# Frank-Wang-oss/GNN_RUL_Benchmarking

Measured on AMD Instinct MI355X. Metric: training samples/sec, C-MAPSS FD004-shaped ST_GCN, higher is better.
Workload: dtype f32 (f16x2-split MFMA operands, fp32 accumulate); 1 GPU; ST_GCN.update (fwd+MSE+bwd+Adam), C-MAPSS FD004-shaped windows [14 sensors x 30], per-GPU batch 65536, dropout 0.2, lr 0.0001, wd 0.0001; per_gpu_batch=65536, global_batch=65536, num_patch=14, patch_size=30, parallelism=dp1, batchnorm=single process, loss_readback=end of run (device-side loss each step)

## Files before the change

gnn_rul_benchmarking_amd/csrc/stgcn_train.hip:

```cpp
#include "stgcn_device.hpp"
#include "stgcn_host.hpp"
#include "stgcn_train_layout.hpp"
#include "stgcn_train_mx.hpp"

namespace rulgnn {


constexpr int TT_STRIDE = 68;
constexpr int TT_ROWS = 30;
constexpr int CONVT_FLOATS = F * 2 * F;
constexpr int BNC = 7;

enum PhaseKind { PH_F = 0, PH_TOP = 1, PH_G = 2 };
constexpr int PHASE_WAVES_F1 = 5, PHASE_WAVES_F2 = 4, PHASE_WAVES_TOP = 3, PHASE_WAVES_G1 = 3, PHASE_WAVES_G0 = 3;

template <int L>
struct SavedSlot {
    static constexpr int X(int l) { return l - 1; }
    static constexpr int H(int l) { return (L - 1) + l; }
    static constexpr int Z1(int l) { return (L - 1) + L + l; }
    static constexpr int O0(int l) { return (L - 1) + 2 * L + l; }
    static constexpr int Z2(int l) { return (L - 1) + 3 * L + l; }
};
static inline int saved_slots(int L) { return 5 * L - 1; }
// ... 1323 lines not shown
    f.gpart = k.gpart; f.cells = k.cells;
    f.grads = a->grads; f.loss = a->loss; f.bn_batch = a->bn_batch;
    f.grid_top = (int)grid;
    for (int i = 0; i < 16; ++i) f.grid_g[i] = (int)grid;
    f.N = k.N; f.L = L; f.K = 1; f.pcount = k.pcount; f.B = s->batch; f.global_batch = a->global_batch;
    f.moment_weight = a->bn_moment_weight;
    f.cell_grad_scale = 1.0f;
    f.guard = 0;
    f.fused_opt = fused_adam ? 1 : 0;
    f.params = fused_adam ? opt->params : nullptr; f.exp_avg = fused_adam ? opt->exp_avg : nullptr;
    f.exp_avg_sq = fused_adam ? opt->exp_avg_sq : nullptr; f.bn_running = fused_adam ? opt->bn_stats : nullptr;
    f.beta1 = fused_adam ? opt->beta1 : 0.f; f.beta2 = fused_adam ? opt->beta2 : 0.f; f.eps = fused_adam ? opt->eps : 0.f;
    f.weight_decay = fused_adam ? opt->weight_decay : 0.f; f.bn_momentum = fused_adam ? opt->bn_momentum : 0.f;
    f.write_grads = 1;
    f.write_loss = (k.has_dpred == 0) && a->loss;
    const float* gy = a->dpred ? a->dpred : a->y;
    if (hipMemsetAsync(c.barrier, 0, sizeof(unsigned), stream) != hipSuccess) return RULGNN_EHIP;
    (void)hipGetLastError();
    hipLaunchKernelGGL(kern, dim3((unsigned)grid), dim3(BLOCK), lds, stream, a->x, a->params, gy, k, c);
    return hipGetLastError() == hipSuccess ? RULGNN_OK : RULGNN_EHIP;
}

template <int RW, int L>
static int run_train_coop(const rulgnn_stgcn_shape* s, const rulgnn_stgcn_train_args* a, hipStream_t stream, const TrainK& k,
                          const WsLayout& w, const TileGeom& g, const rulgnn_adam_args* opt, double bn_count) {
    if constexpr (RW == 16 && L == 2) {
        if (k.N == 14 && k.P == 30) return launch_coop<RW, L, 14, 30>(s, a, stream, k, w, g, opt, bn_count);
        if (k.N == 14 && k.P == 50) return launch_coop<RW, L, 14, 50>(s, a, stream, k, w, g, opt, bn_count);
    }
    return launch_coop<RW, L, 0, 0>(s, a, stream, k, w, g, opt, bn_count);
}

template <int L>
static MxTrainArgs mx_args(const rulgnn_stgcn_shape* s, const rulgnn_stgcn_train_args* a, const TrainK& k, bool wide = false) {
    MxTrainArgs m;
    const size_t tile_floats = wide ? (size_t)F * 64 : (size_t)F * 4 * k.N;
    m.prm = a->params; m.y = a->y; m.pred = a->pred; m.cells = k.cells; m.gpart = k.gpart;
    m.xrec[0] = k.cacheX;
    m.qrec[0] = nullptr;
    for (int l = 0; l < 3; ++l)
        m.mrec[l] = l < L ? reinterpret_cast<uint32_t*>(k.saved + (size_t)SavedSlot<L>::O0(l) * k.ntiles * tile_floats) : nullptr;
    for (int l = 0; l < 3; ++l) m.hrec[l] = l < L ? k.saved + (size_t)SavedSlot<L>::Z1(l) * k.ntiles * tile_floats : nullptr;
    for (int l = 1; l < 3; ++l) {
        m.xrec[l] = l < L ? k.saved + (size_t)SavedSlot<L>::X(l) * k.ntiles * tile_floats : nullptr;
        m.qrec[l] = l < L ? k.saved + (size_t)SavedSlot<L>::Z2(l - 1) * k.ntiles * tile_floats : nullptr;
    }
    m.arec = k.cacheA;
    m.sb = k.sbuf; m.dx = k.rbuf;
    m.dtop = k.saved + (size_t)SavedSlot<L>::H(0) * k.ntiles * tile_floats;
    m.B = s->batch; m.global_batch = a->global_batch; m.sample_offset = a->sample_offset;
    m.N = k.N; m.L = L; m.pcount = k.pcount;
    m.dropout_p = k.dropout_p; m.drop_scale = k.drop_scale; m.drop_thr = k.drop_thr;
    m.do_backward = k.do_backward;
    return m;
}
template <int L>
static int mx_phase(const rulgnn_stgcn_shape* s, const rulgnn_stgcn_train_args* a, const TrainK& k, const MxTrainArgs& m, int ph,
                    hipStream_t stream, int max_grid, int* grid_out, bool wide = false, const HeadScalars* head = nullptr) {
    if (wide) {
        if (ph == 0) return stgcn_train_mxw_f0(m, a->x, s->patch_size, stream, head);
        if (ph < 2 * L) return stgcn_train_mxw_phase(m, PH_F, ph, stream, max_grid, grid_out);
        if (ph == 2 * L) return stgcn_train_mxw_phase(m, PH_TOP, 0, stream, max_grid, grid_out);
        return stgcn_train_mxw_phase(m, PH_G, 4 * L - ph, stream, max_grid, grid_out);
    }
    if (ph == 0)
        return stgcn_train_f0_mx_packed(s, a->x, a->params, m.xrec[0], m.arec, k.cells + cell_fwd(L), cell_stride(L), CELL_REPLICAS, stream, head);
    if (ph < 2 * L) return stgcn_train_mx_phase(m, PH_F, ph, stream, max_grid, grid_out);
    if (ph == 2 * L) return stgcn_train_mx_phase(m, PH_TOP, 0, stream, max_grid, grid_out);
    return stgcn_train_mx_phase(m, PH_G, 4 * L - ph, stream, max_grid, grid_out);
}

template <int RW, int L>
static int run_train_rw(const rulgnn_stgcn_shape* s, const rulgnn_stgcn_train_args* a, int mode, hipStream_t stream,
                        TrainK& k, WsLayout& w, TileGeom& lds, const rulgnn_adam_args* opt, const SyncHook* hook, int path) {
    int rc = RULGNN_OK;
// ... 218 lines not shown
```

gnn_rul_benchmarking_amd/csrc/stgcn_train_mx.hip:

```cpp
#include <algorithm>
#include <cstdlib>
#include <type_traits>

#include "stgcn_host.hpp"
#include "stgcn_mx.hpp"
#include "stgcn_train_layout.hpp"
#include "stgcn_train_mx.hpp"
#include "stgcn_train_mx_ops.hpp"

namespace rulgnn {

#ifdef MXP_TRACE
__device__ unsigned mxp_ts[128];
__device__ int mxp_n;
__device__ unsigned mxp_id[128];
#define MXP_MARKI(ID) do { if (blockIdx.x == 0 && threadIdx.x == 0 && mxp_n < 128) { mxp_id[mxp_n] = ID; mxp_ts[mxp_n++] = (unsigned)wall_clock64(); } } while (0)
#define MXP_MARK() MXP_MARKI(0)
__device__ __forceinline__ void mxp_dump() {
    if (blockIdx.x == 0 && threadIdx.x == 0) {
        for (int i = 0; i < mxp_n; ++i) {
            if (mxp_id[i] >= 100) printf("\nphase %u:", mxp_id[i]);
            else printf(" [%u] +%u", mxp_id[i], mxp_ts[i] - mxp_ts[i - 1]);
        }
        printf("\n");
        mxp_n = 0;
    }
}
#else
#define MXP_MARK() do {} while (0)
#define MXP_MARKI(ID) do {} while (0)
#endif
template <int L, int KIND, int IDX, int NFIX, bool PERSIST>
__device__ __forceinline__ void mxt_phase_body(const MxTrainK& a, float* smem_all, unsigned target) {
    MXP_MARKI(100 + KIND * 10 + IDX);
    const int N = NFIX ? NFIX : a.N;
    const int LS = layer_stride(N);
    const int lane = threadIdx.x & 63, wave = threadIdx.x >> 6;
    const int g = lane >> 4, col = lane & 15;
    constexpr int NBN = 2 * L;
    constexpr int CS = cell_stride(L);
    constexpr int LY = KIND == PH_TOP ? L - 1 : IDX / 2;
    constexpr int BLK = KIND == PH_TOP ? 1 : IDX % 2;
    constexpr bool WITH_PREV = KIND == PH_F && BLK == 0 && LY >= 1;
    constexpr bool BWD_PREV = KIND == PH_G && BLK == 0 && LY >= 1;
    constexpr int LIN = WITH_PREV ? LY - 1 : LY;
    constexpr bool GRAD_IN = KIND == PH_G && (BLK == 1 || LY >= 1);
    constexpr bool GRAD_TOP = GRAD_IN && LY == L - 1;
    constexpr bool NEED_SB = KIND == PH_G && BLK == 0;
    constexpr bool H_OUT = KIND == PH_F && WITH_PREV;
    constexpr bool H_IN = (KIND == PH_F || KIND == PH_G) && BLK == 1 && LY >= 1;
    constexpr bool H_TOP = KIND == PH_TOP && LY >= 1;
    static_assert(!(KIND == PH_F && IDX == 0), "F_0 is stgcn_train_f0_mx_kernel");

    const int XF = 40 * N;
    constexpr int AF = H_IN ? 0 : 220;
    constexpr int SH_BNC = (NBN * MXT_BNC * F + 3) & ~3;
    float* const bnc = smem_all;
    float* const red = smem_all + SH_BNC;
    double* const pairbuf = reinterpret_cast<double*>(red + MXT_RED_FLOATS);
    const int off_zero = 0;
    const int off_scr = off_zero + MXT_ZERO_FLOATS;
    const int off_sh = off_scr + MXT_SCRATCH_FLOATS;
    const int off_wg = off_sh + MXT_SHIFT_FLOATS;
    const int off_X = off_wg + (KIND == PH_G ? MXT_WG_FLOATS : 0);
    const int off_A = off_X + XF;
    const int off_SB = off_A + (H_TOP ? XF : AF);
    const int off_DX = off_SB + (NEED_SB ? XF : 0);
    const int off_XP = off_DX + (GRAD_IN ? XF : 0);
    const int off_HS = off_XP + (BWD_PREV ? XF : 0);
    const int wave_floats = off_HS + (H_OUT ? XF : 0);
    float* const smem = smem_all + SH_BNC + MXT_RED_FLOATS + 2 * MXT_WAVES * (2 * F + 2) + wave * wave_floats;
    u32x2* const sh_tile = reinterpret_cast<u32x2*>(smem + off_sh);
    u32x2* const wg_img = reinterpret_cast<u32x2*>(smem + off_wg);

    int64_t tile = (int64_t)blockIdx.x * MXT_WAVES + wave;
    const int64_t tstride = (int64_t)gridDim.x * MXT_WAVES;

    auto dma = [&](const float* src, int off, int bytes) {
        if constexpr (NFIX != 0) {
            if (bytes == 160 * NFIX) { dma_tile_fixed<160 * NFIX>(src, smem + off, lane); return; }
            if (bytes == 32 * NFIX) { dma_tile_fixed<32 * NFIX>(src, smem + off, lane); return; }
        }
        if constexpr (AF != 0) {
            if (bytes == 4 * AF) { dma_tile_fixed<4 * AF>(src, smem + off, lane); return; }
        }
        dma_tile(src, smem + off, bytes, lane);
    };
    auto req_XA = [&](int64_t t) {
        if constexpr (H_IN) {
            dma(a.hrec[LY] + t * XF, off_X, 4 * XF);
        } else if constexpr (H_TOP) {
            dma(a.xrec[LIN] + t * XF, off_X, 4 * XF);
            dma(a.hrec[LY] + t * XF, off_A, 4 * XF);
        } else {
            dma(a.xrec[LIN] + t * XF, off_X, 4 * XF);
            dma(a.arec + t * AF, off_A, 4 * AF);
        }
    };
    auto req_SB = [&](int64_t t) { if constexpr (NEED_SB) dma(a.sb + t * XF, off_SB, 4 * XF); };
    auto req_DX = [&](int64_t t) {
        if constexpr (GRAD_TOP) dma(a.dtop + t * (8 * N), off_DX, 32 * N);
        else if constexpr (GRAD_IN) dma(a.dx + t * XF, off_DX, 4 * XF);
    };
    auto req_XP = [&](int64_t t) { if constexpr (BWD_PREV) dma(a.qrec[LY] + t * XF, off_XP, 4 * XF); };

    constexpr int FW0 = WITH_PREV ? 2 * LY - 2 : 2 * LY;
    constexpr int NFW = (KIND == PH_F && BLK == 1) || (KIND == PH_G && BLK == 0) ? 1 : 2;
    static_assert(NFW + (KIND == PH_G ? 1 : 0) <= MXT_WAVES, "one reduction pair per wavefront");
    const bool bn_fwd = wave < NFW, bn_mine = bn_fwd || (KIND == PH_G && wave == NFW);
    const int bn_b = bn_fwd ? FW0 + wave : IDX;
    BnPairRaw bnraw;
    if (!PERSIST && bn_mine) bn_pair_load<false>(bnraw, a.cells, a.prm, L, N, bn_fwd, bn_b, lane);
    __builtin_amdgcn_sched_barrier(0);
    for (int i = lane; i < MXT_ZERO_FLOATS; i += 64) smem[off_zero + i] = 0.f;
    if (lane < 2) sh_tile[64 + 65 * lane] = u32x2{0u, 0u};
    if constexpr (KIND == PH_G) {
        if (lane < 2) wg_img[WG_H_HI + WG_ZERO + (WG_H_LO - WG_H_HI) * lane] = u32x2{0u, 0u};
    }
    constexpr int M0_LY = (KIND == PH_F && BLK == 0) ? 1 : 2;
    constexpr int M1_LY = (KIND == PH_F && BLK == 0) ? 0 : ((KIND == PH_F) ? 1 : ((KIND == PH_G && BLK == 0) ? 0 : 2));
    MXP_MARKI(1);
    LayerRaw rc, rp;
    layer_raw(rc, a.prm, LY, N, g, col, M0_LY, M1_LY, !(H_IN || H_TOP));
    if constexpr (WITH_PREV) layer_raw(rp, a.prm, LY - 1, N, g, col, 2, 2);
    ConvOp wT = ConvOp{u32x4{0u, 0u, 0u, 0u}, u32x4{0u, 0u, 0u, 0u}};
    ThetaOp thN = ThetaOp{u32x4{0u, 0u, 0u, 0u}, u32x4{0u, 0u, 0u, 0u}};
    ConvRaw wT_raw = ConvRaw{{0.f, 0.f, 0.f, 0.f}, {0.f, 0.f, 0.f, 0.f}};
    ThetaRaw thN_raw = ThetaRaw{{0.f, 0.f, 0.f, 0.f}};
    if constexpr (KIND == PH_G) {
        wT_raw = conv_bwd_raw(a.prm + LY * LS + off_conv_w(N, BLK), g, col);
        if constexpr (BLK == 0 && LY >= 1) thN_raw = theta_n_raw(a.prm + LY * LS, N, g, col);
    }
    float fc1w[16], fc1wT[16];
    float fc1b = 0.f, fc2w = 0.f, fc2b = 0.f;
    if constexpr (KIND == PH_TOP) {
        const int colc = col < N ? col : 0;
#pragma unroll
        for (int k = 0; k < 16; ++k) {
            const int kc2 = k < N ? k : 0;
            const float v = a.prm[off_fc1_w(N, L) + colc * N + kc2], vt = a.prm[off_fc1_w(N, L) + kc2 * N + colc];
            fc1w[k] = (col < N && k < N) ? v : 0.f;
            fc1wT[k] = (col < N && k < N) ? vt : 0.f;
        }
        const float b1 = a.prm[off_fc1_b(N, L) + colc], w2 = a.prm[off_fc2_w(N, L) + colc];
        fc1b = col < N ? b1 : 0.f;
        fc2w = col < N ? w2 : 0.f;
        fc2b = a.prm[off_fc2_b(N, L)];
    }
    uint32_t dkey[L];
#pragma unroll
    for (int l = 0; l < L; ++l) dkey[l] = step_scratch(a.cells, L)->drop_key[l];
    const bool use_drop = a.dropout_p > 0.f;
    uint32_t mask_next = 0u;
    constexpr bool MASK_IN = KIND == PH_G && BLK == 1;
    if constexpr (MASK_IN) {
        if (use_drop && tile < a.ntiles) mask_next = a.mrec[LY][tile * 64 + lane];
    }
    __builtin_amdgcn_sched_barrier(0);
    if (tile < a.ntiles) { req_XA(tile); req_SB(tile); req_DX(tile); req_XP(tile); }
    {
        MXP_MARKI(2);
        if constexpr (PERSIST) {
            if (threadIdx.x == 0) {
                unsigned* const ctr = step_barrier(a.cells, L);
                unsigned spins = 0;
                while (__hip_atomic_load(ctr, __ATOMIC_RELAXED, __HIP_MEMORY_SCOPE_AGENT) < target) {
                    __builtin_amdgcn_s_sleep(1);
                    if (++spins > (1u << 22)) { atomicOr(&step_scratch(a.cells, L)->pad[0], 4u); break; }
                }
            }
            __syncthreads();
        }
        constexpr bool COH = PERSIST;
        MXP_MARKI(3);
        if (bn_mine) {
            if constexpr (PERSIST) bn_pair_load<COH>(bnraw, a.cells, a.prm, L, N, bn_fwd, bn_b, lane);
            bn_pair_finish(bnraw, bnc, bn_fwd, bn_b, lane);
        }
        if constexpr (KIND == PH_G) {
            wT = conv_bwd_pack(wT_raw);
            if constexpr (BLK == 0 && LY >= 1) thN = theta_pack(thN_raw);
        }
        __syncthreads();
    }
    MXP_MARKI(4);
    LayerK kc;
    layer_constants(kc, rc, bnc, LY, g, col, M0_LY, M1_LY);
    LayerK kp;
    if constexpr (WITH_PREV) layer_constants(kp, rp, bnc, LY - 1, g, col, 2, 2);
    float bA[3] = {0.f, 0.f, 0.f}, bk1[3] = {0.f, 0.f, 0.f}, bk2[3] = {0.f, 0.f, 0.f};
    if constexpr (KIND == PH_G) {
        const float* q = bnc + IDX * MXT_BNC * F;
#pragma unroll
        for (int r = 0; r < 3; ++r) {
            const int c = slot_chan(4 * g + r);
            bA[r] = c >= 0 ? q[4 * F + c] : 0.f;
            bk1[r] = c >= 0 ? q[5 * F + c] * a.gscale : 0.f;
            bk2[r] = c >= 0 ? q[6 * F + c] * a.gscale : 0.f;
        }
    }

    const bool col_ok = col < N;
    const float colm = col_ok ? 1.f : 0.f;
    const int pitch = 4 * N;
    int xoff[3], aoff[3], chan[3];
#pragma unroll
    for (int r = 0; r < 3; ++r) {
        const int c = slot_chan(4 * g + r);
        chan[r] = c;
        xoff[r] = (c >= 0 && col_ok) ? c * pitch + col : -1;
    }
    {
        const int cc = slot_chan(col);
#pragma unroll
        for (int r = 0; r < 3; ++r) {
            const int c = slot_chan(4 * g + r);
            aoff[r] = (c >= 0 && cc >= 0) ? sym(c, cc) : -1;
        }
    }
    auto ld_tile = [&](int base, float (&v)[4][3]) {
#pragma unroll
        for (int s = 0; s < 4; ++s)
// ... 65 lines not shown
        __builtin_amdgcn_sched_barrier(0);
    };
    auto stage_conv = [&](const auto& D, float partner, const ConvOp& w, int rd, int rd_lo, auto& z, auto& keep, auto& keep_sh) {
        constexpr int NS = std::extent_v<std::remove_reference_t<decltype(z)>>;
        u32x4 bh[NS], bl[NS];
#pragma unroll
        for (int s = 0; s < NS; ++s) {
            const Pk p = pack3(D[s][0], D[s][1], D[s][2], partner);
            const Shifted prev = shift_read(sh_tile, rd, rd_lo, lane, p);
            bh[s] = cat(p.hi, prev.hi);
            bl[s] = cat(p.lo, prev.lo);
            keep[s] = p;
            keep_sh[s] = prev;
            __builtin_amdgcn_sched_barrier(0);
        }
        __builtin_amdgcn_sched_barrier(0);
#pragma unroll
        for (int s = 0; s < NS; ++s) {
            z[s] = mfma16z(w.hi, bh[s]);
            z[s] = mfma16(w.hi, bl[s], z[s]);
            z[s] = mfma16(w.lo, bh[s], z[s]);
        }
        __builtin_amdgcn_sched_barrier(0);
    };
    auto leaky_of = [&](const auto& Hp, auto& H) {
        constexpr int NS = std::extent_v<std::remove_reference_t<decltype(H)>>;
#pragma unroll
        for (int s = 0; s < NS; ++s) {
            keep_until_here(Hp[s][3]);
#pragma unroll
            for (int r = 0; r < 3; ++r) H[s][r] = fmaf((1.f - LEAKY) / (1.f + LEAKY), __builtin_fabsf(Hp[s][r]), Hp[s][r]);
        }
    };
    auto layer_full = [&](float (&X)[4][3], const u32x4 (&adjB)[4], const LayerK& k, uint32_t key, const uint32_t (&sbase)[4],
                          float (*xh1_out)[4][3], float (*y2_out)[4][3], float (*q_out)[4][3], uint32_t* mbits_out,
                          const float (*h_in)[4][3] = nullptr) {
        f32x4 z[4];
        float H[4][3], V[4][3];
        Pk pk[4];
        Shifted ps[4];
        if (h_in) {
#pragma unroll
            for (int s = 0; s < 4; ++s)
#pragma unroll
                for (int r = 0; r < 3; ++r) H[s][r] = (*h_in)[s][r];
        } else {
            f32x4 T[4], Hp[4];
            Op2 xo[4];
            stage_T(X, adjB, T, xo);
            stage_Hp(T, k.th, Hp);
            leaky_of(Hp, H);
        }
        stage_conv(H, 1.0f, k.w[0], sh_rd1, sh_rd1_lo, z, pk, ps);
#pragma unroll
        for (int s = 0; s < 4; ++s) {
            keep_until_here(z[s][3]);
#pragma unroll
            for (int r = 0; r < 3; ++r) {
                const float y1 = fmaf(k.gam[0][r], z[s][r], k.bet[0][r]);
                V[s][r] = relu2(fmaf(2.f, H[s][r], relu2(y1)));
            }
        }
        stage_conv(V, 1.0f, k.w[1], sh_rd2, sh_rd2_lo, z, pk, ps);
        uint32_t mbits = 0u;
#pragma unroll
        for (int s = 0; s < 4; ++s) {
            keep_until_here(z[s][3]);
#pragma unroll
            for (int r = 0; r < 3; ++r) {
                const float xh = z[s][r];
                const float y2 = fmaf(k.gam[1][r], xh, k.bet[1][r]);
                if (xh1_out) (*xh1_out)[s][r] = xh;
                if (y2_out) (*y2_out)[s][r] = y2;
                float o1 = fmaf(0.5f, relu2(y2), 0.25f * V[s][r]);
                bool keep = true;
                if (use_drop) {
                    const uint32_t h = lowbias32((sbase[s] + dro[r]) ^ key);
                    keep = h >= a.drop_thr;
                    o1 = keep ? o1 * a.drop_scale : 0.f;
                    mbits |= keep ? 1u << (3 * s + r) : 0u;
                }
                if (q_out) (*q_out)[s][r] = (keep && y2 > 0.f) ? xh : INFINITY;
                X[s][r] = fmaf(colm, o1, X[s][r]);
            }
        }
        *mbits_out = mbits;
    };

    bool pend = false;
    int64_t pend_tile = 0;
    int pend_ns = 0;
    float pend_v[4][3], pend_q[4][3], pend_h[4][3];
    float pend_top0 = 0.f, pend_top1 = 0.f, pend_pred = 0.f;
    uint32_t pend_m = 0u;
#pragma unroll
    for (int s = 0; s < 4; ++s)
#pragma unroll
        for (int r = 0; r < 3; ++r) pend_v[s][r] = pend_q[s][r] = pend_h[s][r] = 0.f;

    MXP_MARKI(5);
    for (; tile < a.ntiles; tile += tstride) {
        const int64_t s0 = tile * 4;
        const int ns_tile = (int)((a.B - s0) < 4 ? (a.B - s0) : 4);
        auto tile_body = [&](auto FULL_) {
        constexpr bool FULL = decltype(FULL_)::value;
        const int ns = FULL ? 4 : ns_tile;
        const int64_t nt = tile + tstride;
        asm volatile("s_waitcnt vmcnt(0) lgkmcnt(0)" ::: "memory");
        __builtin_amdgcn_wave_barrier();
        if (!pend) MXP_MARKI(13);
        if (pend) {
            if constexpr (WITH_PREV) {
                st_tile(a.xrec[LY] + pend_tile * XF, pend_v, pend_ns);
                st_tile(a.qrec[LY] + pend_tile * XF, pend_q, pend_ns);
                if (use_drop) a.mrec[LY - 1][pend_tile * 64 + lane] = pend_m;
            }
            if constexpr (H_OUT) st_tile_staged(a.hrec[LY] + pend_tile * XF, pend_h);
            if constexpr (KIND == PH_G && BLK == 1) st_tile(a.sb + pend_tile * XF, pend_v, pend_ns);
            if constexpr (BWD_PREV) st_tile(a.dx + pend_tile * XF, pend_v, pend_ns);
            if constexpr (KIND == PH_TOP) {
                if (g < pend_ns && col_ok && a.do_backward) {
                    float* p = a.dtop + pend_tile * (8 * N) + g * N + col;
                    p[0] = pend_top0;
                    p[pitch] = pend_top1;
                }
                if (g < pend_ns && col == 0) a.pred[pend_tile * 4 + g] = pend_pred;
                if (use_drop && a.do_backward) a.mrec[LY][pend_tile * 64 + lane] = pend_m;
            }
        }
        float X[4][3];
        float HT[4][3];
        u32x4 adjB[4];
        ld_tile(off_X, X);
        if constexpr (H_TOP) ld_tile(off_A, HT);
        if constexpr (H_IN || H_TOP) {
            if (ns < 4) {
#pragma unroll
                for (int s = 0; s < 4; ++s)
                    if (s >= ns) {
                        X[s][0] = X[s][1] = X[s][2] = 0.f;
                        if constexpr (H_TOP) HT[s][0] = HT[s][1] = HT[s][2] = 0.f;
                    }
            }
        } else {
#pragma unroll
            for (int s = 0; s < 4; ++s) {
                unsigned q[3];
#pragma unroll
                for (int r = 0; r < 3; ++r) q[r] = __builtin_bit_cast(unsigned, smem[(aoff[r] >= 0 ? off_A + aoff[r] : off_zero) + s * 55]);
                adjB[s] = u32x4{__builtin_amdgcn_perm(q[1], q[0], 0x05040100u), q[2] & 0xFFFFu, __builtin_amdgcn_perm(q[1], q[0], 0x07060302u), q[2] >> 16};
            }
            if (ns < 4) {
#pragma unroll
                for (int s = 0; s < 4; ++s)
                    if (s >= ns) { adjB[s] = u32x4{0u, 0u, 0u, 0u}; X[s][0] = X[s][1] = X[s][2] = 0.f; }
            }
        }
        asm volatile("s_waitcnt lgkmcnt(0)" ::: "memory");
        __builtin_amdgcn_wave_barrier();
        if (nt < a.ntiles) req_XA(nt);
        uint32_t sbase[4];
#pragma unroll
        for (int s = 0; s < 4; ++s) sbase[s] = (uint32_t)((a.sample_offset + s0 + s) * F) * (uint32_t)N;
        const bool any_row = true;
        (void)any_row;

        if constexpr (KIND == PH_F) {
            if constexpr (WITH_PREV) {
                layer_full(X, adjB, kp, dkey[LY - 1], sbase, nullptr, nullptr, &pend_q, &pend_m);
#pragma unroll
                for (int s = 0; s < 4; ++s)
#pragma unroll
                    for (int r = 0; r < 3; ++r) pend_v[s][r] = X[s][r];
            }
            f32x4 z[4];
            float H[4][3];
            Pk pk[4];
            Shifted ps[4];
            if constexpr (H_IN) {
#pragma unroll
                for (int s = 0; s < 4; ++s)
#pragma unroll
                    for (int r = 0; r < 3; ++r) H[s][r] = X[s][r];
            } else {
                f32x4 T[4], Hp[4];
                Op2 xo[4];
                stage_T(X, adjB, T, xo);
                stage_Hp(T, kc.th, Hp);
                leaky_of(Hp, H);
            }
            if constexpr (H_OUT) {
#pragma unroll
                for (int s = 0; s < 4; ++s)
#pragma unroll
                    for (int r = 0; r < 3; ++r) pend_h[s][r] = H[s][r];
            }
            if constexpr (BLK == 0) {
                stage_conv(H, 0.f, kc.w[0], sh_rd1, sh_rd1_lo, z, pk, ps);
            } else {
                stage_conv(H, 1.0f, kc.w[0], sh_rd1, sh_rd1_lo, z, pk, ps);
                float V[4][3];
#pragma unroll
                for (int s = 0; s < 4; ++s) {
                    keep_until_here(z[s][3]);
#pragma unroll
                    for (int r = 0; r < 3; ++r) V[s][r] = relu2(fmaf(2.f, H[s][r], relu2(fmaf(kc.gam[0][r], z[s][r], kc.bet[0][r]))));
                }
                stage_conv(V, 0.f, kc.w[1], sh_rd2, sh_rd2_lo, z, pk, ps);
            }
#pragma unroll
            for (int s = 0; s < 4; ++s) {
                keep_until_here(z[s][3]);
                if (s < ns) {
#pragma unroll
                    for (int r = 0; r < 3; ++r) {
                        const float zv = z[s][r] * colm;
                        s_a[r] += zv;
                        s_b[r] = fmaf(zv, zv, s_b[r]);
                    }
                }
            }
            if constexpr (H_OUT) { pend = true; pend_tile = tile; pend_ns = ns; }
            return;
        }

        if constexpr (KIND == PH_TOP) {
            float xh1[4][3], y2[4][3];
            const float ylab = a.y[s0 + (g < ns ? g : ns - 1)];
            if constexpr (H_TOP) layer_full(X, adjB, kc, dkey[LY], sbase, &xh1, &y2, nullptr, &pend_m, &HT);
            else layer_full(X, adjB, kc, dkey[LY], sbase, &xh1, &y2, nullptr, &pend_m);
            float pm[4], pa[4];
#pragma unroll
            for (int s = 0; s < 4; ++s) {
                const float v0 = X[s][0], v1 = g == 3 ? X[s][0] : X[s][1], v2 = g == 3 ? X[s][0] : X[s][2];
                float m = v0;
                int ar = 0;
                if (v1 > m) { m = v1; ar = 1; }
                if (v2 > m) { m = v2; ar = 2; }
                pm[s] = fmaf(v0 + v1 + v2, 0.f, m);
                pa[s] = __builtin_bit_cast(float, 3 * g + ar);
            }
            transpose_rows4(pm[0], pm[1], pm[2], pm[3]);
            transpose_rows4(pa[0], pa[1], pa[2], pa[3]);
            float pooled = pm[0];
            int arg = __builtin_bit_cast(int, pa[0]);
#pragma unroll
            for (int q = 1; q < 4; ++q) {
                const bool take = pm[q] > pooled;
                pooled = take ? pm[q] : pooled;
                arg = take ? __builtin_bit_cast(int, pa[q]) : arg;
            }
            pooled = fmaf((pm[0] + pm[1]) + (pm[2] + pm[3]), 0.f, pooled);
            const bool rowok = g < ns, valid = rowok && col_ok;
            pooled = valid ? pooled : 0.f;
            float y1 = fc1b;
            fmac1_rowbcast<0>(y1, pooled, fc1w[0]);   fmac1_rowbcast<1>(y1, pooled, fc1w[1]);   fmac1_rowbcast<2>(y1, pooled, fc1w[2]);
            fmac1_rowbcast<3>(y1, pooled, fc1w[3]);   fmac1_rowbcast<4>(y1, pooled, fc1w[4]);   fmac1_rowbcast<5>(y1, pooled, fc1w[5]);
            fmac1_rowbcast<6>(y1, pooled, fc1w[6]);   fmac1_rowbcast<7>(y1, pooled, fc1w[7]);   fmac1_rowbcast<8>(y1, pooled, fc1w[8]);
            fmac1_rowbcast<9>(y1, pooled, fc1w[9]);   fmac1_rowbcast<10>(y1, pooled, fc1w[10]); fmac1_rowbcast<11>(y1, pooled, fc1w[11]);
            fmac1_rowbcast<12>(y1, pooled, fc1w[12]); fmac1_rowbcast<13>(y1, pooled, fc1w[13]); fmac1_rowbcast<14>(y1, pooled, fc1w[14]);
            fmac1_rowbcast<15>(y1, pooled, fc1w[15]);
            y1 = relu(y1);
            const float pred = Row<16>::allsum(y1 * fc2w) + fc2b;
// ... 255 lines not shown
                        for (int e = 0; e < NS; ++e) {
                            keep_until_here(dXl[e][3]);
#pragma unroll
                            for (int r = 0; r < 3; ++r) {
                                const float dX = (HS + e < ns) ? (dXl[e][r] + gin[HS + e][r]) * colm : 0.f;
                                pend_v[HS + e][r] = dX;
                                const bool open = Q[HS + e][r] < INFINITY;
                                const float dy = open ? dX * a.drop_scale : 0.f;
                                s_a[r] += dy;
                                s_b[r] = fmaf(dy, open ? Q[HS + e][r] : 0.f, s_b[r]);
                            }
                        }
                    }
                }
            };
            g_half(std::integral_constant<int, 0>{});
            __builtin_amdgcn_sched_barrier(0);
            g_half(std::integral_constant<int, 2>{});
            if constexpr (BLK == 1 || LY >= 1) { pend = true; pend_tile = tile; pend_ns = ns; }
        }
        };
        if (ns_tile == 4) tile_body(std::true_type{});
        else tile_body(std::false_type{});
    }

    MXP_MARKI(6);
    if (pend) {
        if constexpr (WITH_PREV) {
            st_tile(a.xrec[LY] + pend_tile * XF, pend_v, pend_ns);
            st_tile(a.qrec[LY] + pend_tile * XF, pend_q, pend_ns);
            if (use_drop) a.mrec[LY - 1][pend_tile * 64 + lane] = pend_m;
        }
        if constexpr (H_OUT) st_tile_staged(a.hrec[LY] + pend_tile * XF, pend_h);
        if constexpr (KIND == PH_G && BLK == 1) st_tile(a.sb + pend_tile * XF, pend_v, pend_ns);
        if constexpr (BWD_PREV) st_tile(a.dx + pend_tile * XF, pend_v, pend_ns);
        if constexpr (KIND == PH_TOP) {
            if (g < pend_ns && col_ok && a.do_backward) {
                float* p = a.dtop + pend_tile * (8 * N) + g * N + col;
                p[0] = pend_top0;
                p[pitch] = pend_top1;
            }
            if (g < pend_ns && col == 0) a.pred[pend_tile * 4 + g] = pend_pred;
            if (use_drop && a.do_backward) a.mrec[LY][pend_tile * 64 + lane] = pend_m;
        }
    }

    MXP_MARKI(7);
    StepScratch* const sc = step_scratch(a.cells, L);
    bool bad = false;
    const bool has_pair = (KIND == PH_F) || (KIND == PH_TOP && a.do_backward) || (KIND == PH_G && IDX > 0);
    constexpr int PBW = 2 * F + 2;
    if (has_pair) {
#pragma unroll
        for (int r = 0; r < 3; ++r) {
            double da = (double)s_a[r], db = (double)s_b[r];
#pragma unroll
            for (int off = 8; off >= 1; off >>= 1) {
                da += __shfl_xor(da, off, 16);
                db += __shfl_xor(db, off, 16);
            }
            if (col == 0 && chan[r] >= 0) {
                pairbuf[wave * PBW + chan[r]] = da;
                pairbuf[wave * PBW + F + chan[r]] = db;
            }
        }
    }
// ... 104 lines not shown
    asm volatile("s_waitcnt vmcnt(0) lgkmcnt(0)" ::: "memory");
    MXP_MARKI(12);
    __syncthreads();
    if (threadIdx.x == 0) __hip_atomic_fetch_add(step_barrier(a.cells, L), 1u, __ATOMIC_RELAXED, __HIP_MEMORY_SCOPE_AGENT);
    ++arrived_phases;
}
template <int L, int NFIX, int I>
struct MxtPersistChain {
    static __device__ __forceinline__ void forward(const MxTrainK& a, float* smem_all, unsigned& n) {
        if constexpr (I > 1) MxtPersistChain<L, NFIX, I - 1>::forward(a, smem_all, n);
        mxt_persist_phase<L, PH_F, I, NFIX>(a, smem_all, n);
    }
    static __device__ __forceinline__ void backward(const MxTrainK& a, float* smem_all, unsigned& n) {
        mxt_persist_phase<L, PH_G, I, NFIX>(a, smem_all, n);
        if constexpr (I > 0) MxtPersistChain<L, NFIX, I - 1>::backward(a, smem_all, n);
    }
};
template <int L, int NFIX>
__global__ __launch_bounds__(64 * MXT_WAVES, MX_WAVES_PER_SIMD) void stgcn_train_mx_persist_kernel(MxTrainK a) {
    extern __shared__ __attribute__((aligned(16))) float smem_all[];
    unsigned n = 0;
    MxtPersistChain<L, NFIX, 2 * L - 1>::forward(a, smem_all, n);
    mxt_persist_phase<L, PH_TOP, 0, NFIX>(a, smem_all, n);
    MxtPersistChain<L, NFIX, 2 * L - 1>::backward(a, smem_all, n);
#ifdef MXP_TRACE
    mxp_dump();
#endif
}

static constexpr size_t mxt_lds_bytes(int L, int kind, int idx, int N) {
    const int blk = kind == PH_TOP ? 1 : idx % 2, ly = kind == PH_TOP ? L - 1 : idx / 2;
    const bool need_sb = kind == PH_G && blk == 0, grad_in = kind == PH_G && (blk == 1 || ly >= 1), bwd_prev = kind == PH_G && blk == 0 && ly >= 1;
    const bool h_in = (kind == PH_F || kind == PH_G) && blk == 1 && ly >= 1;
    const bool h_top = kind == PH_TOP && ly >= 1;
    const bool h_out = kind == PH_F && blk == 0 && ly >= 1;
    const int XF = 40 * N;
    const size_t wave = (size_t)MXT_ZERO_FLOATS + MXT_SCRATCH_FLOATS + MXT_SHIFT_FLOATS + (kind == PH_G ? MXT_WG_FLOATS : 0) + XF + (h_in ? 0 : h_top ? XF : 220) + (need_sb ? XF : 0) + (grad_in ? XF : 0) +
                        (bwd_prev ? XF : 0) + (h_out ? XF : 0);
    const size_t shared = (size_t)((2 * L * MXT_BNC * F + 3) & ~3) + MXT_RED_FLOATS + 2 * MXT_WAVES * (2 * F + 2);
    return (shared + MXT_WAVES * wave) * sizeof(float);
}
constexpr size_t MXT_MAX_LDS_BYTES = 80 * 1024;
static_assert(mxt_lds_bytes(MX_MAX_LAYERS, PH_G, 2, 15) <= MXT_MAX_LDS_BYTES && mxt_lds_bytes(MX_MAX_LAYERS, PH_G, 3, 15) <= MXT_MAX_LDS_BYTES,
              "the largest matrix-core phase must fit its LDS limit");

template <int L, int KIND, int IDX, int NFIX>
static int mxt_launch(const MxTrainK& k, hipStream_t stream, int max_grid, int* grid_out) {
    auto kern = &stgcn_train_mx_kernel<L, KIND, IDX, NFIX>;
    const size_t lds = mxt_lds_bytes(L, KIND, IDX, k.N);
    if (lds > MXT_MAX_LDS_BYTES) return RULGNN_EUNSUPPORTED;
    if (lds > 48 * 1024 &&
        hipFuncSetAttribute(reinterpret_cast<const void*>(kern), hipFuncAttributeMaxDynamicSharedMemorySize, (int)lds) != hipSuccess)
        return RULGNN_EHIP;
    int dev = 0, cus = 256, per_cu = 0;
    if (hipGetDevice(&dev) == hipSuccess) {
        int v = 0;
        if (hipDeviceGetAttribute(&v, hipDeviceAttributeMultiprocessorCount, dev) == hipSuccess && v > 0) cus = v;
    }
    if (hipOccupancyMaxActiveBlocksPerMultiprocessor(&per_cu, kern, 64 * MXT_WAVES, lds) != hipSuccess || per_cu < 1) per_cu = 1;
    if (per_cu > MX_WAVES_PER_SIMD) per_cu = MX_WAVES_PER_SIMD;
    if (const char* e = getenv("RULGNN_MXT_BLOCKS_PER_CU")) { const int v = atoi(e); if (v > 0) per_cu = v; }
    int64_t grid = (int64_t)cus * per_cu;
    const int64_t want = (k.ntiles + MXT_WAVES - 1) / MXT_WAVES;
    if (grid > want) grid = want;
    if (grid > max_grid) grid = max_grid;
    if (grid_out) *grid_out = (int)grid;
    (void)hipGetLastError();
    hipLaunchKernelGGL(kern, dim3((unsigned)grid), dim3(64 * MXT_WAVES), lds, stream, k);
    return hipGetLastError() == hipSuccess ? RULGNN_OK : RULGNN_EHIP;
}

// ... 4 lines not shown
}

template <int L, int I>
struct MxtPhase {
    static int run(int kind, int idx, const MxTrainK& k, hipStream_t st, int mg, int* go) {
        if (idx == I) {
            if (kind == PH_F) {
                if constexpr (I >= 1) return mxt_launch_n<L, PH_F, I>(k, st, mg, go);
                else return RULGNN_EINVAL;
            }
            if (kind == PH_G) return mxt_launch_n<L, PH_G, I>(k, st, mg, go);
        }
        if constexpr (I > 0) return MxtPhase<L, I - 1>::run(kind, idx, k, st, mg, go);
        return RULGNN_EINVAL;
    }
};

bool stgcn_train_mx_shape_ok(const rulgnn_stgcn_shape* s, const float* x) {
    const int N = s->num_patch, P = s->patch_size, L = s->num_layers;
    if (N < 2 || N > 15 || L < 1 || L > MX_MAX_LAYERS || s->mpnn_k != 1) return false;
    if (((int64_t)N * P) % 4 != 0 || (reinterpret_cast<uintptr_t>(x) & 15) != 0) return false;
    return true;
}

float stgcn_train_mx_grad_scale(int64_t global_batch) {
    int e = 0;
    while (((int64_t)1 << e) < global_batch && e < 40) ++e;
    return ldexpf(1.0f, e + 3);
}

static MxTrainK mxt_kernel_args(const MxTrainArgs& m) {
    MxTrainK k;
    k.prm = m.prm; k.y = m.y; k.pred = m.pred; k.cells = m.cells; k.gpart = m.gpart;
    for (int l = 0; l < MX_MAX_LAYERS; ++l) { k.xrec[l] = m.xrec[l]; k.qrec[l] = m.qrec[l]; k.hrec[l] = m.hrec[l]; k.mrec[l] = m.mrec[l]; }
    k.arec = m.arec; k.sb = m.sb; k.dx = m.dx; k.dtop = m.dtop;
    k.B = m.B; k.ntiles = (m.B + 3) / 4; k.global_batch = m.global_batch; k.sample_offset = m.sample_offset;
    k.N = m.N; k.pcount = m.pcount;
    k.dropout_p = m.dropout_p; k.drop_scale = m.drop_scale; k.drop_thr = m.drop_thr;
    k.gscale = stgcn_train_mx_grad_scale(m.global_batch);
    k.inv_gscale = 1.0f / k.gscale;
    k.do_backward = m.do_backward;
    return k;
}

template <int NFIX>
static int mxt_persist_launch(const MxTrainK& k, hipStream_t stream, int64_t grid) {
    constexpr int L = 2;
    auto kern = &stgcn_train_mx_persist_kernel<L, NFIX>;
    size_t lds = 0;
    for (int i = 1; i < 2 * L; ++i) lds = std::max(lds, mxt_lds_bytes(L, PH_F, i, k.N));
    lds = std::max(lds, mxt_lds_bytes(L, PH_TOP, 0, k.N));
    for (int i = 0; i < 2 * L; ++i) lds = std::max(lds, mxt_lds_bytes(L, PH_G, i, k.N));
    if (lds > MXT_MAX_LDS_BYTES) return RULGNN_EUNSUPPORTED;
    if (lds > 48 * 1024 &&
        hipFuncSetAttribute(reinterpret_cast<const void*>(kern), hipFuncAttributeMaxDynamicSharedMemorySize, (int)lds) != hipSuccess)
        return RULGNN_EHIP;
    (void)hipGetLastError();
    hipLaunchKernelGGL(kern, dim3((unsigned)grid), dim3(64 * MXT_WAVES), lds, stream, k);
    return hipGetLastError() == hipSuccess ? RULGNN_OK : RULGNN_EHIP;
}
int stgcn_train_mx_persistent_grid(int64_t batch, int num_layers, int max_grid) {
    if (num_layers != 2 || batch <= 0) return 0;
    int dev = 0, cus = 256;
    if (hipGetDevice(&dev) == hipSuccess) {
        int v = 0;
        if (hipDeviceGetAttribute(&v, hipDeviceAttributeMultiprocessorCount, dev) == hipSuccess && v > 0) cus = v;
    }
// ... 33 lines not shown
```

gnn_rul_benchmarking_amd/csrc/stgcn_train_mx.hpp:

```cpp
#pragma once
#include <hip/hip_runtime.h>
#include <stdint.h>

#include "../../include/rulgnn.h"

namespace rulgnn {

struct MxTrainArgs {
    const float* prm;
    const float* y;
    float* pred;
    double* cells;
    float* gpart;
    float* xrec[3];
    float* qrec[3];
    float* hrec[3];
    uint32_t* mrec[3];
    float* arec;
    float* sb;
    float* dx;
    float* dtop;
    int64_t B, global_batch, sample_offset;
    int N, L, pcount;
    float dropout_p, drop_scale;
    uint32_t drop_thr;
    int do_backward;
};

bool stgcn_train_mx_shape_ok(const rulgnn_stgcn_shape* s, const float* x);
float stgcn_train_mx_grad_scale(int64_t global_batch);
int stgcn_train_mx_phase(const MxTrainArgs& m, int kind, int idx, hipStream_t stream, int max_grid, int* grid_out);
int stgcn_train_mx_persistent_grid(int64_t batch, int num_layers, int max_grid);
int stgcn_train_mx_persistent(const MxTrainArgs& m, hipStream_t stream, int max_grid, int* grid_out);
struct HeadScalars;
int stgcn_train_f0_mx_packed(const rulgnn_stgcn_shape* s, const float* x, const float* prm, float* xrec0, float* arec, double* cells_bn0,
                             int cell_stride_doubles, int replicas, hipStream_t stream, const HeadScalars* head = nullptr);


bool stgcn_train_mxw_shape_ok(const rulgnn_stgcn_shape* s, const float* x);
int stgcn_train_mxw_f0(const MxTrainArgs& m, const float* x, int patch_size, hipStream_t stream, const HeadScalars* head = nullptr);
int stgcn_train_mxw_phase(const MxTrainArgs& m, int kind, int idx, hipStream_t stream, int max_grid, int* grid_out);

}
```

gnn_rul_benchmarking_amd/csrc/stgcn_train_mx_ops.hpp:

```cpp
#pragma once
#include <type_traits>

#include "stgcn_mx.hpp"
#include "stgcn_train_layout.hpp"

namespace rulgnn {
namespace {

constexpr int MXT_ZERO_FLOATS = 192;
constexpr int MXT_SCRATCH_FLOATS = 128;
constexpr int MXT_SHIFT_FLOATS = 264;
constexpr int WG_ZERO = 64;
constexpr int WG_DZ_HI = 0, WG_DZ_LO = 64, WG_H_HI = 128, WG_H_LO = WG_H_HI + 65;
constexpr int MXT_WG_FLOATS = (2 * (WG_H_LO + 65) + 3) & ~3;
constexpr int MXT_WAVES = 4;
constexpr int MXT_RED_FLOATS = 448;
constexpr int MXT_BNC = BN_TABLE_ROWS;

enum { PH_F = 0, PH_TOP = 1, PH_G = 2 };

struct Op2 { u32x4 h, l; };
struct Pk { u32x2 hi, lo; };

__device__ __forceinline__ Pk pack3(float a, float b, float c, float d) {
// ... 117 lines not shown
    }
}
__device__ __forceinline__ void layer_constants(LayerK& k, const LayerRaw& raw, const float* bnc, int l, int g, int col, int mode0, int mode1) {
    k.th = theta_pack(raw.th);
    const int co = slot_chan(col), coc = co >= 0 ? co : 0;
#pragma unroll
    for (int blk = 0; blk < 2; ++blk) {
        const int mode = blk == 0 ? mode0 : mode1;
        const float* q = bnc + (2 * l + blk) * MXT_BNC * F;
        const float istd = mode == 2 ? q[1 * F + coc] : 1.f;
        const float shift = mode == 2 ? -q[0 * F + coc] * istd : 0.f;
        if (mode != 0) k.w[blk] = conv_fwd_operand(raw.w[blk], istd, shift, blk == 0 ? 1.f : 0.25f, g, col);
        else k.w[blk] = ConvOp{u32x4{0u, 0u, 0u, 0u}, u32x4{0u, 0u, 0u, 0u}};
#pragma unroll
        for (int r = 0; r < 3; ++r) {
            const int c = slot_chan(4 * g + r);
            k.gam[blk][r] = (mode == 2 && c >= 0) ? q[2 * F + c] : 0.f;
            k.bet[blk][r] = (mode == 2 && c >= 0) ? q[3 * F + c] : 0.f;
        }
    }
}

}

struct MxTrainK {
    const float* prm;
    const float* y;
    float* pred;
    double* cells;
    float* gpart;
    float* xrec[MX_MAX_LAYERS];
    float* qrec[MX_MAX_LAYERS];
    float* hrec[MX_MAX_LAYERS];
    uint32_t* mrec[MX_MAX_LAYERS];
    float* arec;
    float* sb;
    float* dx;
    float* dtop;
    int64_t B, ntiles, global_batch, sample_offset;
    int N, pcount;
    float dropout_p, drop_scale;
    uint32_t drop_thr;
    float gscale, inv_gscale;
    int do_backward;
};

}
```

Measured before the change: 207.5 million samples/s.

## Store block-1 conv input per layer and reload it instead of recomputing

```diff
diff --git a/gnn_rul_benchmarking_amd/csrc/stgcn_train.hip b/gnn_rul_benchmarking_amd/csrc/stgcn_train.hip
--- a/gnn_rul_benchmarking_amd/csrc/stgcn_train.hip
+++ b/gnn_rul_benchmarking_amd/csrc/stgcn_train.hip
@@ -1379,6 +1379,21 @@
 }
 
 template <int L>
+constexpr int mx_orec_slot(int l) { return l < L - 1 ? SavedSlot<L>::H(l + 1) : SavedSlot<L>::Z2(L - 1); }
+template <int L>
+constexpr bool mx_orec_slots_free() {
+    for (int l = 0; l < L; ++l) {
+        const int v = mx_orec_slot<L>(l);
+        if (v < 0 || v >= 5 * L - 1 || v == SavedSlot<L>::H(0)) return false;
+        for (int j = 0; j < L; ++j) {
+            if (v == SavedSlot<L>::Z1(j) || v == SavedSlot<L>::O0(j) || (j != l && v == mx_orec_slot<L>(j))) return false;
+            if (j >= 1 && (v == SavedSlot<L>::X(j) || v == SavedSlot<L>::Z2(j - 1))) return false;
+        }
+    }
+    return true;
+}
+static_assert(mx_orec_slots_free<1>() && mx_orec_slots_free<2>() && mx_orec_slots_free<3>(), "the o0 record must not share a slot");
+template <int L>
 static MxTrainArgs mx_args(const rulgnn_stgcn_shape* s, const rulgnn_stgcn_train_args* a, const TrainK& k, bool wide = false) {
     MxTrainArgs m;
     const size_t tile_floats = wide ? (size_t)F * 64 : (size_t)F * 4 * k.N;
@@ -1388,6 +1403,7 @@
     for (int l = 0; l < 3; ++l)
         m.mrec[l] = l < L ? reinterpret_cast<uint32_t*>(k.saved + (size_t)SavedSlot<L>::O0(l) * k.ntiles * tile_floats) : nullptr;
     for (int l = 0; l < 3; ++l) m.hrec[l] = l < L ? k.saved + (size_t)SavedSlot<L>::Z1(l) * k.ntiles * tile_floats : nullptr;
+    for (int l = 0; l < 3; ++l) m.orec[l] = (l < L && !wide) ? k.saved + (size_t)mx_orec_slot<L>(l) * k.ntiles * tile_floats : nullptr;
     for (int l = 1; l < 3; ++l) {
         m.xrec[l] = l < L ? k.saved + (size_t)SavedSlot<L>::X(l) * k.ntiles * tile_floats : nullptr;
         m.qrec[l] = l < L ? k.saved + (size_t)SavedSlot<L>::Z2(l - 1) * k.ntiles * tile_floats : nullptr;
diff --git a/gnn_rul_benchmarking_amd/csrc/stgcn_train_mx.hip b/gnn_rul_benchmarking_amd/csrc/stgcn_train_mx.hip
--- a/gnn_rul_benchmarking_amd/csrc/stgcn_train_mx.hip
+++ b/gnn_rul_benchmarking_amd/csrc/stgcn_train_mx.hip
@@ -49,7 +49,8 @@
     constexpr bool NEED_SB = KIND == PH_G && BLK == 0;
     constexpr bool H_OUT = KIND == PH_F && WITH_PREV;
     constexpr bool H_IN = (KIND == PH_F || KIND == PH_G) && BLK == 1 && LY >= 1;
-    constexpr bool H_TOP = KIND == PH_TOP && LY >= 1;
+    constexpr bool V_OUT = KIND == PH_F && BLK == 1;
+    constexpr bool V_TOP = KIND == PH_TOP;
     static_assert(!(KIND == PH_F && IDX == 0), "F_0 is stgcn_train_f0_mx_kernel");
 
     const int XF = 40 * N;
@@ -64,11 +65,12 @@
     const int off_wg = off_sh + MXT_SHIFT_FLOATS;
     const int off_X = off_wg + (KIND == PH_G ? MXT_WG_FLOATS : 0);
     const int off_A = off_X + XF;
-    const int off_SB = off_A + (H_TOP ? XF : AF);
+    const int off_SB = off_A + (V_TOP ? XF : AF);
     const int off_DX = off_SB + (NEED_SB ? XF : 0);
     const int off_XP = off_DX + (GRAD_IN ? XF : 0);
-    const int off_HS = off_XP + (BWD_PREV ? XF : 0);
-    const int wave_floats = off_HS + (H_OUT ? XF : 0);
+    const int off_V = off_XP + (BWD_PREV ? XF : 0);
+    const int off_HS = off_V + (WITH_PREV ? XF : 0);
+    const int wave_floats = off_HS + ((H_OUT || V_OUT) ? XF : 0);
     float* const smem = smem_all + SH_BNC + MXT_RED_FLOATS + 2 * MXT_WAVES * (2 * F + 2) + wave * wave_floats;
     u32x2* const sh_tile = reinterpret_cast<u32x2*>(smem + off_sh);
     u32x2* const wg_img = reinterpret_cast<u32x2*>(smem + off_wg);
@@ -89,12 +91,13 @@
     auto req_XA = [&](int64_t t) {
         if constexpr (H_IN) {
             dma(a.hrec[LY] + t * XF, off_X, 4 * XF);
-        } else if constexpr (H_TOP) {
+        } else if constexpr (V_TOP) {
             dma(a.xrec[LIN] + t * XF, off_X, 4 * XF);
-            dma(a.hrec[LY] + t * XF, off_A, 4 * XF);
+            dma(a.orec[LY] + t * XF, off_A, 4 * XF);
         } else {
             dma(a.xrec[LIN] + t * XF, off_X, 4 * XF);
             dma(a.arec + t * AF, off_A, 4 * AF);
+            if constexpr (WITH_PREV) dma(a.orec[LIN] + t * XF, off_V, 4 * XF);
         }
     };
     auto req_SB = [&](int64_t t) { if constexpr (NEED_SB) dma(a.sb + t * XF, off_SB, 4 * XF); };
@@ -104,8 +107,8 @@
     };
     auto req_XP = [&](int64_t t) { if constexpr (BWD_PREV) dma(a.qrec[LY] + t * XF, off_XP, 4 * XF); };
 
-    constexpr int FW0 = WITH_PREV ? 2 * LY - 2 : 2 * LY;
-    constexpr int NFW = (KIND == PH_F && BLK == 1) || (KIND == PH_G && BLK == 0) ? 1 : 2;
+    constexpr int FW0 = WITH_PREV ? 2 * LY - 1 : (V_TOP ? 2 * LY + 1 : 2 * LY);
+    constexpr int NFW = KIND == PH_G && BLK == 1 ? 2 : 1;
     static_assert(NFW + (KIND == PH_G ? 1 : 0) <= MXT_WAVES, "one reduction pair per wavefront");
     const bool bn_fwd = wave < NFW, bn_mine = bn_fwd || (KIND == PH_G && wave == NFW);
     const int bn_b = bn_fwd ? FW0 + wave : IDX;
@@ -117,12 +120,12 @@
     if constexpr (KIND == PH_G) {
         if (lane < 2) wg_img[WG_H_HI + WG_ZERO + (WG_H_LO - WG_H_HI) * lane] = u32x2{0u, 0u};
     }
-    constexpr int M0_LY = (KIND == PH_F && BLK == 0) ? 1 : 2;
+    constexpr int M0_LY = (KIND == PH_F && BLK == 0) ? 1 : (V_TOP ? 0 : 2);
     constexpr int M1_LY = (KIND == PH_F && BLK == 0) ? 0 : ((KIND == PH_F) ? 1 : ((KIND == PH_G && BLK == 0) ? 0 : 2));
     MXP_MARKI(1);
     LayerRaw rc, rp;
-    layer_raw(rc, a.prm, LY, N, g, col, M0_LY, M1_LY, !(H_IN || H_TOP));
-    if constexpr (WITH_PREV) layer_raw(rp, a.prm, LY - 1, N, g, col, 2, 2);
+    layer_raw(rc, a.prm, LY, N, g, col, M0_LY, M1_LY, !(H_IN || V_TOP));
+    if constexpr (WITH_PREV) layer_raw(rp, a.prm, LY - 1, N, g, col, 0, 2, false);
     ConvOp wT = ConvOp{u32x4{0u, 0u, 0u, 0u}, u32x4{0u, 0u, 0u, 0u}};
     ThetaOp thN = ThetaOp{u32x4{0u, 0u, 0u, 0u}, u32x4{0u, 0u, 0u, 0u}};
     ConvRaw wT_raw = ConvRaw{{0.f, 0.f, 0.f, 0.f}, {0.f, 0.f, 0.f, 0.f}};
@@ -187,7 +190,7 @@
     LayerK kc;
     layer_constants(kc, rc, bnc, LY, g, col, M0_LY, M1_LY);
     LayerK kp;
-    if constexpr (WITH_PREV) layer_constants(kp, rp, bnc, LY - 1, g, col, 2, 2);
+    if constexpr (WITH_PREV) layer_constants(kp, rp, bnc, LY - 1, g, col, 0, 2);
     float bA[3] = {0.f, 0.f, 0.f}, bk1[3] = {0.f, 0.f, 0.f}, bk2[3] = {0.f, 0.f, 0.f};
     if constexpr (KIND == PH_G) {
         const float* q = bnc + IDX * MXT_BNC * F;
@@ -319,35 +322,11 @@
             for (int r = 0; r < 3; ++r) H[s][r] = fmaf((1.f - LEAKY) / (1.f + LEAKY), __builtin_fabsf(Hp[s][r]), Hp[s][r]);
         }
     };
-    auto layer_full = [&](float (&X)[4][3], const u32x4 (&adjB)[4], const LayerK& k, uint32_t key, const uint32_t (&sbase)[4],
-                          float (*xh1_out)[4][3], float (*y2_out)[4][3], float (*q_out)[4][3], uint32_t* mbits_out,
-                          const float (*h_in)[4][3] = nullptr) {
+    auto layer_tail = [&](float (&X)[4][3], const float (&V)[4][3], const LayerK& k, uint32_t key, const uint32_t (&sbase)[4],
+                          float (*xh1_out)[4][3], float (*y2_out)[4][3], float (*q_out)[4][3], uint32_t* mbits_out) {
         f32x4 z[4];
-        float H[4][3], V[4][3];
         Pk pk[4];
         Shifted ps[4];
-        if (h_in) {
-#pragma unroll
-            for (int s = 0; s < 4; ++s)
-#pragma unroll
-                for (int r = 0; r < 3; ++r) H[s][r] = (*h_in)[s][r];
-        } else {
-            f32x4 T[4], Hp[4];
-            Op2 xo[4];
-            stage_T(X, adjB, T, xo);
-            stage_Hp(T, k.th, Hp);
-            leaky_of(Hp, H);
-        }
-        stage_conv(H, 1.0f, k.w[0], sh_rd1, sh_rd1_lo, z, pk, ps);
-#pragma unroll
-        for (int s = 0; s < 4; ++s) {
-            keep_until_here(z[s][3]);
-#pragma unroll
-            for (int r = 0; r < 3; ++r) {
-                const float y1 = fmaf(k.gam[0][r], z[s][r], k.bet[0][r]);
-                V[s][r] = relu2(fmaf(2.f, H[s][r], relu2(y1)));
-            }
-        }
         stage_conv(V, 1.0f, k.w[1], sh_rd2, sh_rd2_lo, z, pk, ps);
         uint32_t mbits = 0u;
 #pragma unroll
@@ -403,6 +382,7 @@
                 if (use_drop) a.mrec[LY - 1][pend_tile * 64 + lane] = pend_m;
             }
             if constexpr (H_OUT) st_tile_staged(a.hrec[LY] + pend_tile * XF, pend_h);
+            if constexpr (V_OUT) st_tile_staged(a.orec[LY] + pend_tile * XF, pend_h);
             if constexpr (KIND == PH_G && BLK == 1) st_tile(a.sb + pend_tile * XF, pend_v, pend_ns);
             if constexpr (BWD_PREV) st_tile(a.dx + pend_tile * XF, pend_v, pend_ns);
             if constexpr (KIND == PH_TOP) {
@@ -416,18 +396,23 @@
             }
         }
         float X[4][3];
-        float HT[4][3];
+        float VR[4][3];
         u32x4 adjB[4];
         ld_tile(off_X, X);
-        if constexpr (H_TOP) ld_tile(off_A, HT);
-        if constexpr (H_IN || H_TOP) {
+        if constexpr (V_TOP) ld_tile(off_A, VR);
+        if constexpr (WITH_PREV) ld_tile(off_V, VR);
+        if constexpr (V_TOP || WITH_PREV) {
             if (ns < 4) {
 #pragma unroll
                 for (int s = 0; s < 4; ++s)
-                    if (s >= ns) {
-                        X[s][0] = X[s][1] = X[s][2] = 0.f;
-                        if constexpr (H_TOP) HT[s][0] = HT[s][1] = HT[s][2] = 0.f;
-                    }
+                    if (s >= ns) VR[s][0] = VR[s][1] = VR[s][2] = 0.f;
+            }
+        }
+        if constexpr (H_IN || V_TOP) {
+            if (ns < 4) {
+#pragma unroll
+                for (int s = 0; s < 4; ++s)
+                    if (s >= ns) X[s][0] = X[s][1] = X[s][2] = 0.f;
             }
         } else {
 #pragma unroll
@@ -454,7 +439,7 @@
 
         if constexpr (KIND == PH_F) {
             if constexpr (WITH_PREV) {
-                layer_full(X, adjB, kp, dkey[LY - 1], sbase, nullptr, nullptr, &pend_q, &pend_m);
+                layer_tail(X, VR, kp, dkey[LY - 1], sbase, nullptr, nullptr, &pend_q, &pend_m);
 #pragma unroll
                 for (int s = 0; s < 4; ++s)
 #pragma unroll
@@ -491,7 +476,7 @@
                 for (int s = 0; s < 4; ++s) {
                     keep_until_here(z[s][3]);
 #pragma unroll
-                    for (int r = 0; r < 3; ++r) V[s][r] = relu2(fmaf(2.f, H[s][r], relu2(fmaf(kc.gam[0][r], z[s][r], kc.bet[0][r]))));
+                    for (int r = 0; r < 3; ++r) pend_h[s][r] = V[s][r] = relu2(fmaf(2.f, H[s][r], relu2(fmaf(kc.gam[0][r], z[s][r], kc.bet[0][r]))));
                 }
                 stage_conv(V, 0.f, kc.w[1], sh_rd2, sh_rd2_lo, z, pk, ps);
             }
@@ -507,15 +492,14 @@
                     }
                 }
             }
-            if constexpr (H_OUT) { pend = true; pend_tile = tile; pend_ns = ns; }
+            if constexpr (H_OUT || V_OUT) { pend = true; pend_tile = tile; pend_ns = ns; }
             return;
         }
 
         if constexpr (KIND == PH_TOP) {
             float xh1[4][3], y2[4][3];
             const float ylab = a.y[s0 + (g < ns ? g : ns - 1)];
-            if constexpr (H_TOP) layer_full(X, adjB, kc, dkey[LY], sbase, &xh1, &y2, nullptr, &pend_m, &HT);
-            else layer_full(X, adjB, kc, dkey[LY], sbase, &xh1, &y2, nullptr, &pend_m);
+            layer_tail(X, VR, kc, dkey[LY], sbase, &xh1, &y2, nullptr, &pend_m);
             float pm[4], pa[4];
 #pragma unroll
             for (int s = 0; s < 4; ++s) {
@@ -837,6 +821,7 @@
             if (use_drop) a.mrec[LY - 1][pend_tile * 64 + lane] = pend_m;
         }
         if constexpr (H_OUT) st_tile_staged(a.hrec[LY] + pend_tile * XF, pend_h);
+        if constexpr (V_OUT) st_tile_staged(a.orec[LY] + pend_tile * XF, pend_h);
         if constexpr (KIND == PH_G && BLK == 1) st_tile(a.sb + pend_tile * XF, pend_v, pend_ns);
         if constexpr (BWD_PREV) st_tile(a.dx + pend_tile * XF, pend_v, pend_ns);
         if constexpr (KIND == PH_TOP) {
@@ -1007,11 +992,12 @@
     const int blk = kind == PH_TOP ? 1 : idx % 2, ly = kind == PH_TOP ? L - 1 : idx / 2;
     const bool need_sb = kind == PH_G && blk == 0, grad_in = kind == PH_G && (blk == 1 || ly >= 1), bwd_prev = kind == PH_G && blk == 0 && ly >= 1;
     const bool h_in = (kind == PH_F || kind == PH_G) && blk == 1 && ly >= 1;
-    const bool h_top = kind == PH_TOP && ly >= 1;
-    const bool h_out = kind == PH_F && blk == 0 && ly >= 1;
+    const bool v_top = kind == PH_TOP;
+    const bool with_prev = kind == PH_F && blk == 0 && ly >= 1;
+    const bool v_out = kind == PH_F && blk == 1;
     const int XF = 40 * N;
-    const size_t wave = (size_t)MXT_ZERO_FLOATS + MXT_SCRATCH_FLOATS + MXT_SHIFT_FLOATS + (kind == PH_G ? MXT_WG_FLOATS : 0) + XF + (h_in ? 0 : h_top ? XF : 220) + (need_sb ? XF : 0) + (grad_in ? XF : 0) +
-                        (bwd_prev ? XF : 0) + (h_out ? XF : 0);
+    const size_t wave = (size_t)MXT_ZERO_FLOATS + MXT_SCRATCH_FLOATS + MXT_SHIFT_FLOATS + (kind == PH_G ? MXT_WG_FLOATS : 0) + XF + (h_in ? 0 : v_top ? XF : 220) + (need_sb ? XF : 0) + (grad_in ? XF : 0) +
+                        (bwd_prev ? XF : 0) + (with_prev ? 2 * XF : 0) + (v_out ? XF : 0);
     const size_t shared = (size_t)((2 * L * MXT_BNC * F + 3) & ~3) + MXT_RED_FLOATS + 2 * MXT_WAVES * (2 * F + 2);
     return (shared + MXT_WAVES * wave) * sizeof(float);
 }
@@ -1082,7 +1068,7 @@
 static MxTrainK mxt_kernel_args(const MxTrainArgs& m) {
     MxTrainK k;
     k.prm = m.prm; k.y = m.y; k.pred = m.pred; k.cells = m.cells; k.gpart = m.gpart;
-    for (int l = 0; l < MX_MAX_LAYERS; ++l) { k.xrec[l] = m.xrec[l]; k.qrec[l] = m.qrec[l]; k.hrec[l] = m.hrec[l]; k.mrec[l] = m.mrec[l]; }
+    for (int l = 0; l < MX_MAX_LAYERS; ++l) { k.xrec[l] = m.xrec[l]; k.qrec[l] = m.qrec[l]; k.hrec[l] = m.hrec[l]; k.orec[l] = m.orec[l]; k.mrec[l] = m.mrec[l]; }
     k.arec = m.arec; k.sb = m.sb; k.dx = m.dx; k.dtop = m.dtop;
     k.B = m.B; k.ntiles = (m.B + 3) / 4; k.global_batch = m.global_batch; k.sample_offset = m.sample_offset;
     k.N = m.N; k.pcount = m.pcount;
diff --git a/gnn_rul_benchmarking_amd/csrc/stgcn_train_mx.hpp b/gnn_rul_benchmarking_amd/csrc/stgcn_train_mx.hpp
--- a/gnn_rul_benchmarking_amd/csrc/stgcn_train_mx.hpp
+++ b/gnn_rul_benchmarking_amd/csrc/stgcn_train_mx.hpp
@@ -15,6 +15,7 @@
     float* xrec[3];
     float* qrec[3];
     float* hrec[3];
+    float* orec[3];
     uint32_t* mrec[3];
     float* arec;
     float* sb;
diff --git a/gnn_rul_benchmarking_amd/csrc/stgcn_train_mx_ops.hpp b/gnn_rul_benchmarking_amd/csrc/stgcn_train_mx_ops.hpp
--- a/gnn_rul_benchmarking_amd/csrc/stgcn_train_mx_ops.hpp
+++ b/gnn_rul_benchmarking_amd/csrc/stgcn_train_mx_ops.hpp
@@ -173,6 +173,7 @@
     float* xrec[MX_MAX_LAYERS];
     float* qrec[MX_MAX_LAYERS];
     float* hrec[MX_MAX_LAYERS];
+    float* orec[MX_MAX_LAYERS];
     uint32_t* mrec[MX_MAX_LAYERS];
     float* arec;
     float* sb;
```

Measured after the change: 203.7 million samples/s. 0.982x the previous value.
